# vliu15/3d-brain-tumor-segmentation

Measured on AMD Instinct MI355X. Metric: training volumes/sec (2ch x 128^3), higher is better.
Workload: dtype f32; 1 GPU; BASELINE configs[1]: 2ch x 128^3, batch 1 per GPU, fp32, full fwd+bwd with Dice+KL+L2 VAE loss + Dice metric + TF-form Adam; CLI-default model (base_filters=32, depth=4, groups=8, reduction=8; 42,174,773 params); parallelism=dp1, global_batch=1

## Files before the change

3d-brain-tumor-segmentation_amd/csrc/conv_wgrad.hip:

```cpp
#include <stdlib.h>
#include <type_traits>
#include "common.h"
#include "bts_internal.h"

#define WG_THREADS 512
#define WG_WAVES 8
#define WG_MAXT 4
#define WG_PSLOTS 8
#define WG_QSLOTS 4

struct WgradParams {
  const float* p;
  const float* q;
  float* partial;
  double* partial_b;
  const float* zeros;
  int N, Dp, Hp, Wp, Cp, ldp;
  int Dq, Hq, Wq, Cq, ldq;
  int s, loz, loy, lox;
  int IZ, IY, IX;
  int lgTX, lgTY, TZ;
  int ntz, nty, ntx;
  int ntaps, ntiles, cpad, lgSP;
  int nsub, sub_per_wg;
// ... 467 lines not shown
      float* dst = p.partial + tileBase + (long)(wave + WG_WAVES * i) * 1024;
#pragma unroll
      for (int r = 0; r < 16; ++r) dst[((r & 3) + 8 * (r >> 2) + 4 * h) * 32 + l32] = acc[i][r];
    }
#pragma unroll
    for (int i = 0; i < 3; ++i) {
      __syncthreads();
#pragma unroll
      for (int r = 0; r < 16; ++r) lds[wave * 1024 + ((r & 3) + 8 * (r >> 2) + 4 * h) * 32 + l32] = accx[i][r];
      __syncthreads();
      float* dst = p.partial + tileBase + (long)(24 + i) * 1024;
      for (int e = tid; e < 1024; e += WG_THREADS) {
        float s = lds[e];
#pragma unroll
        for (int w = 1; w < WG_WAVES; ++w) s += lds[w * 1024 + e];
        dst[e] = s;
      }
    }
  } else if (!ksplit) {
#pragma unroll
    for (int i = 0; i < WG_MAXT; ++i) {
      const int tile = wave + WG_WAVES * i;
      if (tile < p.ntiles) {
        float* dst = p.partial + tileBase + (long)tile * 1024;
#pragma unroll
        for (int r = 0; r < 16; ++r) dst[((r & 3) + 8 * (r >> 2) + 4 * h) * 32 + l32] = acc[i][r];
      }
    }
  } else {
#pragma unroll
    for (int i = 0; i < WG_MAXT; ++i) {
      if (i < p.ntiles) {
        __syncthreads();
#pragma unroll
        for (int r = 0; r < 16; ++r) lds[wave * 1024 + ((r & 3) + 8 * (r >> 2) + 4 * h) * 32 + l32] = acc[i][r];
        __syncthreads();
        float* dst = p.partial + tileBase + (long)i * 1024;
        for (int e = tid; e < 1024; e += WG_THREADS) {
          float s = lds[e];
#pragma unroll
          for (int w = 1; w < WG_WAVES; ++w) s += lds[w * 1024 + e];
          dst[e] = s;
        }
      }
    }
  }
  if (p.want_bias && pct == 0) {
    __syncthreads();
    double* shd = reinterpret_cast<double*>(lds);
    shd[tid] = bsum;
    __syncthreads();
    if (tid < 32) {
      double s = 0.0;
      for (int part = 0; part < 16; ++part) s += shd[part * 32 + tid];
      p.partial_b[((long)blockIdx.x * gridDim.z + qct) * 32 + tid] = s;
    }
  }
}

struct WfinParams {
  const float* partial;
  const double* partial_b;
  float* dw;
  float* db;
  int nsp, npct, nqct, ntaps, ntiles, cpad, Cp, Cq;
  long sT, sP, sQ;
  int fold_axis;
  int shift, dup_start;
  int accum;
};

__global__ __launch_bounds__(256) void wgrad_finalize_kernel(const WfinParams f) {
  __shared__ double sh[32][33];
  const int q4 = threadIdx.x & 7, wl = threadIdx.x >> 3;
  const long rows = (long)f.ntaps * f.Cp * f.nqct;
  const long wgStride = (long)f.npct * f.nqct * f.ntiles * 1024;
  for (long row = blockIdx.x; row < rows; row += gridDim.x) {
    const int qct = (int)(row % f.nqct);
    long r = row / f.nqct;
    const int pc = (int)(r % f.Cp);
    const int t = (int)(r / f.Cp);
    long off;
    if (f.cpad == 32) off = ((((long)(pc >> 5)) * f.nqct + qct) * f.ntiles + t) * 1024 + (pc & 31) * 32;
    else {
      const int ci = t * f.cpad + pc;
      off = ((long)qct * f.ntiles + (ci >> 5)) * 1024 + (ci & 31) * 32;
    }
    const float* src = f.partial + off + q4 * 4;
    double s0 = 0.0, s1 = 0.0, s2 = 0.0, s3 = 0.0;
    int w = wl;
    for (; w + 96 < f.nsp; w += 128) {
      const f32x4 a = *reinterpret_cast<const f32x4*>(src + (long)w * wgStride);
      const f32x4 b = *reinterpret_cast<const f32x4*>(src + (long)(w + 32) * wgStride);
      const f32x4 c = *reinterpret_cast<const f32x4*>(src + (long)(w + 64) * wgStride);
      const f32x4 d = *reinterpret_cast<const f32x4*>(src + (long)(w + 96) * wgStride);
      s0 += (double)a[0]; s1 += (double)a[1]; s2 += (double)a[2]; s3 += (double)a[3];
      s0 += (double)b[0]; s1 += (double)b[1]; s2 += (double)b[2]; s3 += (double)b[3];
      s0 += (double)c[0]; s1 += (double)c[1]; s2 += (double)c[2]; s3 += (double)c[3];
      s0 += (double)d[0]; s1 += (double)d[1]; s2 += (double)d[2]; s3 += (double)d[3];
    }
    for (; w < f.nsp; w += 32) {
      const f32x4 a = *reinterpret_cast<const f32x4*>(src + (long)w * wgStride);
      s0 += (double)a[0]; s1 += (double)a[1]; s2 += (double)a[2]; s3 += (double)a[3];
    }
    __syncthreads();
    sh[wl][q4 * 4 + 0] = s0; sh[wl][q4 * 4 + 1] = s1; sh[wl][q4 * 4 + 2] = s2; sh[wl][q4 * 4 + 3] = s3;
    __syncthreads();
    if (threadIdx.x < 32) {
      const int e = threadIdx.x;
      double totd = sh[0][e];
#pragma unroll
      for (int k = 1; k < 32; ++k) totd += sh[k][e];
      const float tot = (float)totd;
      const int qc = qct * 32 + e;
      if (qc < f.Cq) {
        const int pr = (f.fold_axis == 1) ? pc + f.shift : pc;
        const int qr = (f.fold_axis == 2) ? qc + f.shift : qc;
        float* d1 = f.dw + t * f.sT + pr * f.sP + qr * f.sQ;
        *d1 = f.accum ? (*d1 + tot) : tot;
        if (f.shift > 0) {
          if (f.fold_axis == 1 && pc >= f.dup_start) {
            float* d2 = f.dw + t * f.sT + (pc - f.dup_start) * f.sP + qr * f.sQ;
            *d2 = f.accum ? (*d2 + tot) : tot;
          } else if (f.fold_axis == 2 && qc >= f.dup_start) {
            float* d2 = f.dw + t * f.sT + pr * f.sP + (qc - f.dup_start) * f.sQ;
            *d2 = f.accum ? (*d2 + tot) : tot;
          }
        }
      }
    }
  }
  if (f.db && (int)blockIdx.x < f.nqct) {
    const int e = threadIdx.x & 31, l8 = threadIdx.x >> 5, qct = blockIdx.x;
    double s = 0.0;
    for (int w = l8; w < f.nsp; w += 8) s += f.partial_b[((long)w * f.nqct + qct) * 32 + e];
    __syncthreads();
    sh[l8][e] = s;
    __syncthreads();
    if (l8 == 0 && qct * 32 + e < f.Cq) {
      double tot = sh[0][e];
#pragma unroll
      for (int k = 1; k < 8; ++k) tot += sh[k][e];
      const int i = qct * 32 + e;
      f.db[i] = f.accum ? (f.db[i] + (float)tot) : (float)tot;
    }
  }
}

__global__ __launch_bounds__(256) void wgrad_finalize_flat_kernel(const WfinParams f) {
  const int nq = f.nqct * 32;
  const long total = (long)f.ntaps * f.Cp * nq;
  const long wgStride = (long)f.npct * f.nqct * f.ntiles * 1024;
  for (long i = blockIdx.x * (long)blockDim.x + threadIdx.x; i < total; i += (long)gridDim.x * blockDim.x) {
    const int qc = (int)(i % nq);
    long r = i / nq;
    const int pc = (int)(r % f.Cp);
    const int t = (int)(r / f.Cp);
    if (qc >= f.Cq) continue;
    const int qct = qc >> 5, e = qc & 31;
    long off;
    if (f.cpad == 32) off = ((((long)(pc >> 5)) * f.nqct + qct) * f.ntiles + t) * 1024 + (pc & 31) * 32 + e;
    else {
      const int ci = t * f.cpad + pc;
      off = ((long)qct * f.ntiles + (ci >> 5)) * 1024 + (ci & 31) * 32 + e;
    }
    double totd = 0.0;
    for (int w = 0; w < f.nsp; ++w) totd += (double)f.partial[w * wgStride + off];
    const float tot = (float)totd;
    const int pr = (f.fold_axis == 1) ? pc + f.shift : pc;
    const int qr = (f.fold_axis == 2) ? qc + f.shift : qc;
    float* d1 = f.dw + t * f.sT + pr * f.sP + qr * f.sQ;
    *d1 = f.accum ? (*d1 + tot) : tot;
    if (f.shift > 0) {
      if (f.fold_axis == 1 && pc >= f.dup_start) {
        float* d2 = f.dw + t * f.sT + (pc - f.dup_start) * f.sP + qr * f.sQ;
        *d2 = f.accum ? (*d2 + tot) : tot;
      } else if (f.fold_axis == 2 && qc >= f.dup_start) {
        float* d2 = f.dw + t * f.sT + pr * f.sP + (qc - f.dup_start) * f.sQ;
        *d2 = f.accum ? (*d2 + tot) : tot;
      }
    }
  }
  if (f.db && blockIdx.x == 0) {
    for (int i = threadIdx.x; i < f.Cq; i += blockDim.x) {
      double s = 0.0;
      for (int w = 0; w < f.nsp; ++w) s += f.partial_b[((long)w * f.nqct + (i >> 5)) * 32 + (i & 31)];
      f.db[i] = f.accum ? (f.db[i] + (float)s) : (float)s;
    }
  }
}

static int ilog2w(int v) { int l = 0; while ((1 << l) < v) ++l; return l; }

struct WgCall {
  int kind;
  int N, D, H, W;
  int Cin, ldx, Cout, lddy;
  int dup_shift;
  int want_db;
  int x16, dy16;
};
struct WgradRoles {
  int ntaps, s, neg, swapped, transposed;
  int Dp, Hp, Wp, Cp, Dq, Hq, Wq, Cq;
};
struct WgChoice {
  WgradRoles ro;
  WgradParams p;
  int nsp, npct, nqct;
  size_t shmem;
  int variant;
  int sym;
  long NV;
  double flops;
  int clear_zeros;
  long ws_partial, ws_partial_b, ws_colsum, colsum_bytes, ws_zeros, ws;
};

static int plan_wgrad(WgChoice& pl, int ntaps, int s, int neg, int N, int Dp, int Hp, int Wp_, int Cp, int Dq, int Hq,
                      int Wq, int Cq) {
  WgradParams& p = pl.p;
  p.N = N; p.Dp = Dp; p.Hp = Hp; p.Wp = Wp_; p.Cp = Cp;
  p.Dq = Dq; p.Hq = Hq; p.Wq = Wq; p.Cq = Cq;
  p.s = s; p.ntaps = ntaps;
  int lo = 0, span = 1;
  if (ntaps == 27 && s == 1) { lo = -1; span = 3; }
  if (ntaps == 27 && s == 2) { lo = 0; span = 3; }
  p.loz = p.loy = p.lox = lo;
  int cpad = 32;
  if (Cp <= 16 && ntaps == 27) { cpad = 2; while (cpad < Cp) cpad *= 2; }
  p.cpad = cpad;
  const int SP = cpad == 32 ? 32 : (cpad < 4 ? 4 : cpad);
  p.lgSP = ilog2w(SP);
  p.ntiles = (cpad == 32) ? ntaps : (ntaps * cpad + 31) / 32;
  int TX, TY, TZ;
  if (ntaps == 1) { TX = 32; TY = 4; TZ = 2; }
  else if (s == 1) { TX = 16; TY = 4; TZ = 2; }
  else { TX = 8; TY = 4; TZ = 1; }
  while (TX > 2 && TX / 2 >= Wq) { TX /= 2; if (TY * 2 <= 8) TY *= 2; else TZ *= 2; }
  while (TY > 1 && TY / 2 >= Hq) { TY /= 2; TZ *= 2; }
  while (TZ > 1 && TZ / 2 >= Dq && TX * TY * (TZ / 2) >= 2) TZ /= 2;
  p.lgTX = ilog2w(TX); p.lgTY = ilog2w(TY); p.TZ = TZ;
  p.ntx = (Wq + TX - 1) / TX; p.nty = (Hq + TY - 1) / TY; p.ntz = (Dq + TZ - 1) / TZ;
  p.IX = (TX - 1) * s + span; p.IY = (TY - 1) * s + span; p.IZ = (TZ - 1) * s + span;
  const int tileVoxP = p.IZ * p.IY * p.IX;
  const int M = TX * TY * TZ;
  if (tileVoxP * (SP / 4) > WG_THREADS * WG_PSLOTS || M * 8 > WG_THREADS * WG_QSLOTS) return BTS_ERR_SHAPE;
  pl.shmem = (size_t)2 * ((((tileVoxP * (SP / 4) + 63) & ~63) + ((M * 8 + 63) & ~63)) * 4) * sizeof(float);
  if (pl.shmem < (size_t)WG_WAVES * 1024 * sizeof(float)) pl.shmem = (size_t)WG_WAVES * 1024 * sizeof(float);
  if (pl.shmem > 160 * 1024) return BTS_ERR_SHAPE;
  for (int t = 0; t < 27; ++t) p.tap_vox[t] = 0;
  if (ntaps == 27)
    for (int t = 0; t < 27; ++t) {
      int oz = t / 9 + (s == 1 ? -1 : 0), oy = (t / 3) % 3 + (s == 1 ? -1 : 0), ox = t % 3 + (s == 1 ? -1 : 0);
      if (neg) { oz = -oz; oy = -oy; ox = -ox; }
      p.tap_vox[t] = ((oz - lo) * p.IY + (oy - lo)) * p.IX + (ox - lo);
    }
  p.fixg = 0;
  if (ntaps == 27 && cpad == 32 && !neg) {
    if (s == 1 && TX == 16 && TY == 4 && TZ == 2) p.fixg = 1;
    if (s == 2 && TX == 8 && TY == 4 && TZ == 1) p.fixg = 2;
  }
  p.fastf = 0;
  if (p.fixg && Wq % TX == 0 && Hq % TY == 0 && Dq % TZ == 0 && Cp % 32 == 0 && Cq % 32 == 0)
    p.fastf = 1;
  if (!p.fastf) p.fixg = 0;
  p.nsub = N * p.ntz * p.nty * p.ntx;
  pl.npct = (cpad == 32) ? (Cp + 31) / 32 : 1;
  pl.nqct = (Cq + 31) / 32;
  {
    const long pairs = (long)pl.npct * pl.nqct;
    long best = 1;
    double bestc = 1e30;
    long maxn = 2048 / pairs;
    if (maxn < 1) maxn = 1;
    if (maxn > p.nsub) maxn = p.nsub;
    for (long n = 1; n <= maxn; ++n) {
      const long spw = (p.nsub + n - 1) / n;
      const long ne = (p.nsub + spw - 1) / spw;
      if (ne != n) continue;
      const long rounds = (ne * pairs + 255) / 256;
      const double c = (double)rounds * ((double)spw + 0.5) + 0.0023 * (double)(ne * pairs);
      if (c < bestc - 1e-9) { bestc = c; best = n; }
    }
    if (best > p.nsub) best = p.nsub;
    p.sub_per_wg = (int)((p.nsub + best - 1) / best);
    pl.nsp = (p.nsub + p.sub_per_wg - 1) / p.sub_per_wg;
  }
  return BTS_OK;
}

typedef float wg_f32x2 __attribute__((ext_vector_type(2)));
__device__ __forceinline__ wg_f32x2 wgw_pk_add(wg_f32x2 a, wg_f32x2 b) { wg_f32x2 d; asm("v_pk_add_f32 %0, %1, %2" : "=v"(d) : "v"(a), "v"(b)); return d; }
__device__ __forceinline__ wg_f32x2 wgw_pk_sub(wg_f32x2 a, wg_f32x2 b) { wg_f32x2 d; asm("v_pk_add_f32 %0, %1, %2 neg_lo:[0,1] neg_hi:[0,1]" : "=v"(d) : "v"(a), "v"(b)); return d; }
__device__ __forceinline__ wg_f32x2 wgw_pk_fma(wg_f32x2 a, wg_f32x2 b, wg_f32x2 c) { wg_f32x2 d; asm("v_pk_fma_f32 %0, %1, %2, %3" : "=v"(d) : "v"(a), "v"(b), "v"(c)); return d; }
__device__ __forceinline__ wg_f32x2 wgw_pk_addsub(wg_f32x2 a, wg_f32x2 b) { wg_f32x2 d; asm("v_pk_add_f32 %0, %1, %2 op_sel:[0,1] op_sel_hi:[0,1] neg_hi:[0,1]" : "=v"(d) : "v"(a), "v"(b)); return d; }
__device__ __forceinline__ float wgw_acc_rd(float a) { float v; asm volatile("v_accvgpr_read_b32 %0, %1" : "=v"(v) : "a"(a)); return v; }

#define WGW_THREADS 256
#define WGW_RS 18
#define WGW_PTILE (24 * 32 * WGW_RS)
#define WGW_QTILE (8 * 32 * WGW_RS)
#define WGW_BUF (WGW_PTILE + WGW_QTILE)
#define WGW_NPS 14
#define WGW_NQS 4

__global__ __launch_bounds__(WGW_THREADS, 1) void wgw_kernel(const WgradParams p) {
  extern __shared__ __attribute__((aligned(16))) float lds[];
  const int tid = threadIdx.x;
  const int lane = tid & 63;
  const int wave = __builtin_amdgcn_readfirstlane(tid >> 6);
  const int ch = lane & 31, hh = lane >> 5;
  const int pct = blockIdx.y, qct = blockIdx.z;
  const float* pP = p.p + pct * 32;
  const float* pQ = p.q + qct * 32;

  int p_lds[WGW_NPS];
  unsigned poff[WGW_NPS], pfl[3] = {0u, 0u, 0u};
#pragma unroll
  for (int i = 0; i < WGW_NPS; ++i) {
    const int id = tid + WGW_THREADS * i;
    const int idle = id - 24 * 18 * 8;
    p_lds[i] = WGW_PTILE + ((idle >> 4) * 32 + ((idle >> 1) & 7) * 4) * WGW_RS + 16 + (idle & 1);
    poff[i] = 0x80000000u;
    if (id < 24 * 18 * 8) {
      const int cq = id & 7, vox = id >> 3;
      const int row = vox / 18, xx = vox - row * 18;
      const int zr = row / 6, yr = row - zr * 6;
      p_lds[i] = (row * 32 + cq * 4) * WGW_RS + xx;
      poff[i] = (unsigned)(((zr * p.Hp + yr) * p.Wp + xx) * p.ldp + cq * 4) * 4u;
      const unsigned fl = (zr == 0 ? 1u : 0u) | (zr == 3 ? 2u : 0u) | (yr == 0 ? 4u : 0u) | (yr == 5 ? 8u : 0u) |
                          (xx == 0 ? 16u : 0u) | (xx == 17 ? 32u : 0u);
      pfl[i / 5] |= fl << (6 * (i % 5));
    }
  }
  int q_lds[WGW_NQS];
  unsigned qoff[WGW_NQS];
#pragma unroll
  for (int i = 0; i < WGW_NQS; ++i) {
    const int id = tid + WGW_THREADS * i;
    const int cq = id & 7, xx = (id >> 3) & 15, row = id >> 7;
    q_lds[i] = WGW_PTILE + (row * 32 + cq * 4) * WGW_RS + xx;
    qoff[i] = (unsigned)((((row >> 2) * p.Hq + (row & 3)) * p.Wq + xx) * p.ldq + cq * 4) * 4u;
  }
  const int t0 = blockIdx.x * p.sub_per_wg;
  int t1 = t0 + p.sub_per_wg;
  if (t1 > p.nsub) t1 = p.nsub;
  int ftx, fty, ftz, fn;
  {
    int t = t0;
    ftx = t % p.ntx; t /= p.ntx;
    fty = t % p.nty; t /= p.nty;
    ftz = t % p.ntz;
    fn = t / p.ntz;
  }
  f32x4 pre[WGW_NPS + WGW_NQS];
  __amdgpu_buffer_rsrc_t f_pr, f_qr;
  unsigned f_tm = 0;
  auto fetch_begin = [&](bool live) {
    const int z0 = 2 * ftz, y0 = 4 * fty, x0 = 16 * ftx;
    const float* pb = pP + ((((long)fn * p.Dp + z0 - 1) * p.Hp + y0 - 1) * p.Wp + x0 - 1) * p.ldp;
    const float* qb = pQ + ((((long)fn * p.Dq + z0) * p.Hq + y0) * p.Wq + x0) * p.ldq;
    f_pr = __builtin_amdgcn_make_buffer_rsrc((void*)pb, 0, live ? 0x7fffffff : 0, 0x00020000);
    f_qr = __builtin_amdgcn_make_buffer_rsrc((void*)qb, 0, live ? 0x7fffffff : 0, 0x00020000);
    f_tm = (ftz == 0 ? 1u : 0u) | (ftz == p.ntz - 1 ? 2u : 0u) | (fty == 0 ? 4u : 0u) | (fty == p.nty - 1 ? 8u : 0u) |
           (ftx == 0 ? 16u : 0u) | (ftx == p.ntx - 1 ? 32u : 0u);
    const int cx = (ftx + 1 == p.ntx) ? 1 : 0;
    ftx = cx ? 0 : ftx + 1;
    const int cy = (fty + cx == p.nty) ? 1 : 0;
    fty = cy ? 0 : fty + cx;
    const int cz = (ftz + cy == p.ntz) ? 1 : 0;
    ftz = cz ? 0 : ftz + cy;
    fn += cz;
  };
  auto fetch_slot = [&](auto ic) {
    constexpr int i = decltype(ic)::value;
    if constexpr (i < WGW_NPS) {
      const unsigned fl = ((pfl[i / 5] >> (6 * (i % 5))) & 63u) & f_tm;
      pre[i] = __builtin_bit_cast(f32x4, __builtin_amdgcn_raw_buffer_load_b128(f_pr, fl ? 0x80000000u : poff[i], 0, 0));
    } else {
      pre[i] = __builtin_bit_cast(f32x4, __builtin_amdgcn_raw_buffer_load_b128(f_qr, qoff[i - WGW_NPS], 0, 0));
    }
  };
  auto commit_slot = [&](float* buf, auto ic) {
    constexpr int i = decltype(ic)::value;
    if constexpr (i < WGW_NPS) {
#pragma unroll
      for (int e = 0; e < 4; ++e) buf[p_lds[i] + e * WGW_RS] = pre[i][e];
    } else {
#pragma unroll
      for (int e = 0; e < 4; ++e) buf[q_lds[i - WGW_NPS] + e * WGW_RS] = pre[i][e];
    }
  };
  auto fetch_group = [&](auto kc) {
    constexpr int k = decltype(kc)::value;
    fetch_slot(IC<3 * k>{}); fetch_slot(IC<3 * k + 1>{}); fetch_slot(IC<3 * k + 2>{});
  };
  auto commit_group = [&](float* buf, auto kc) {
    constexpr int k = decltype(kc)::value;
    commit_slot(buf, IC<3 * k>{}); commit_slot(buf, IC<3 * k + 1>{}); commit_slot(buf, IC<3 * k + 2>{});
  };

  const int ra = (wave == 0) ? 0 : (wave == 2) ? 2 : 1;
  const int rb = (wave == 0) ? 2 : (wave == 1) ? 2 : (wave == 2) ? 1 : 3;
  const float sp = (wave == 1) ? 1.f : -1.f;
  const wg_f32x2 sp2 = {sp, sp};
  const float sq = (wave == 1) ? 1.f : (wave == 2) ? -1.f : 0.f;
  const wg_f32x2 sq2 = {sq, sq};
  const int pA = (ra * 6 * 32 + ch) * WGW_RS + 2 * hh, pB = (rb * 6 * 32 + ch) * WGW_RS + 2 * hh;
  const int qXa = WGW_PTILE + ((wave == 3 ? 4 : 0) * 32 + ch) * WGW_RS + 2 * hh;
  const int qYa = WGW_PTILE + (4 * 32 + ch) * WGW_RS + 2 * hh;
  const bool bias = p.want_bias && pct == 0 && wave == 1;
  double bsum = 0.0;
  float bs = 0.f;

  f32x16 acc[4][4];
#pragma unroll
  for (int a = 0; a < 4; ++a)
#pragma unroll
    for (int c = 0; c < 4; ++c)
#pragma unroll
      for (int r = 0; r < 16; ++r) acc[a][c][r] = 0.f;

  struct WgwOps { float v[4][4], t[4][4]; };
  auto form = [&](const float* cur, auto stc, WgwOps& o) {
    constexpr int st = decltype(stc)::value;
    constexpr int py = st >> 2, sx = st & 3;
    wg_f32x2 cl[4], cx[4];
#pragma unroll
    for (int yr = 0; yr < 4; ++yr) {
      const float* a = cur + pA + (2 * py + yr) * 32 * WGW_RS + 4 * sx;
      const float* b = cur + pB + (2 * py + yr) * 32 * WGW_RS + 4 * sx;
      cl[yr] = wgw_pk_fma(*reinterpret_cast<const wg_f32x2*>(b), sp2, *reinterpret_cast<const wg_f32x2*>(a));
      cx[yr] = wgw_pk_fma(*reinterpret_cast<const wg_f32x2*>(b + 2), sp2, *reinterpret_cast<const wg_f32x2*>(a + 2));
    }
    wg_f32x2 vl[4], vx[4];
    vl[0] = wgw_pk_sub(cl[0], cl[2]); vx[0] = wgw_pk_sub(cx[0], cx[2]);
    vl[1] = wgw_pk_add(cl[1], cl[2]); vx[1] = wgw_pk_add(cx[1], cx[2]);
    vl[2] = wgw_pk_sub(cl[2], cl[1]); vx[2] = wgw_pk_sub(cx[2], cx[1]);
    vl[3] = wgw_pk_sub(cl[1], cl[3]); vx[3] = wgw_pk_sub(cx[1], cx[3]);
#pragma unroll
    for (int a = 0; a < 4; ++a) {
      const wg_f32x2 d = wgw_pk_sub(vl[a], vx[a]), m = wgw_pk_addsub(vx[a], vl[a]);
      o.v[a][0] = d.x;
      o.v[a][1] = m.x;
      o.v[a][2] = m.y;
      o.v[a][3] = d.y;
    }
    wg_f32x2 qa[2];
#pragma unroll
    for (int yr = 0; yr < 2; ++yr) {
      const wg_f32x2 X = *reinterpret_cast<const wg_f32x2*>(cur + qXa + (2 * py + yr) * 32 * WGW_RS + 4 * sx);
      const wg_f32x2 Y = *reinterpret_cast<const wg_f32x2*>(cur + qYa + (2 * py + yr) * 32 * WGW_RS + 4 * sx);
      qa[yr] = wgw_pk_fma(Y, sq2, X);
    }
    const wg_f32x2 ty[4] = {qa[0], wgw_pk_add(qa[0], qa[1]), wgw_pk_sub(qa[0], qa[1]), qa[1]};
#pragma unroll
    for (int a = 0; a < 4; ++a) {
      const wg_f32x2 m = wgw_pk_addsub(ty[a], ty[a]);
      o.t[a][0] = ty[a].x;
      o.t[a][1] = m.x;
      o.t[a][2] = m.y;
      o.t[a][3] = ty[a].y;
    }
    bs += o.t[1][1];
  };
  auto mfma16 = [&](const WgwOps& o) {
#pragma unroll
    for (int a = 0; a < 4; ++a)
#pragma unroll
      for (int b = 0; b < 4; ++b) acc[a][b] = __builtin_amdgcn_mfma_f32_32x32x2f32(o.v[a][b], o.t[a][b], acc[a][b], 0, 0, 0);
  };
#define WGW_SCHED_STEP()                                   \
  _Pragma("unroll") for (int q_ = 0; q_ < 16; ++q_) {      \
    __builtin_amdgcn_sched_group_barrier(0x008, 1, 0);     \
    __builtin_amdgcn_sched_group_barrier(0x002, 4, 0);     \
    __builtin_amdgcn_sched_group_barrier(0x320, 3, 0);     \
  }
#define WGW_STEP_END()                       \
  WGW_SCHED_STEP();                          \
  __builtin_amdgcn_sched_barrier(0);         \
  asm volatile("s_nop 1" ::: "memory");

  fetch_begin(t0 < t1);
  fetch_group(IC<0>{}); fetch_group(IC<1>{}); fetch_group(IC<2>{}); fetch_group(IC<3>{}); fetch_group(IC<4>{}); fetch_group(IC<5>{});
  commit_group(lds, IC<0>{}); commit_group(lds, IC<1>{}); commit_group(lds, IC<2>{}); commit_group(lds, IC<3>{});
  commit_group(lds, IC<4>{}); commit_group(lds, IC<5>{});
  __syncthreads();
  WgwOps opA, opB;
  form(lds, IC<0>{}, opA);
  fetch_begin((t0 + 1) < t1);
  __builtin_amdgcn_sched_barrier(0);
  asm volatile("s_nop 3" ::: "memory");
  for (int t = t0; t < t1; ++t) {
    const float* cur = lds + ((t - t0) & 1) * WGW_BUF;
    float* nxt = lds + ((t - t0 + 1) & 1) * WGW_BUF;
    form(cur, IC<1>{}, opB); fetch_group(IC<0>{});
    mfma16(opA);
    WGW_STEP_END();
    form(cur, IC<2>{}, opA); commit_group(nxt, IC<0>{}); fetch_group(IC<1>{});
    mfma16(opB);
    WGW_STEP_END();
    form(cur, IC<3>{}, opB); commit_group(nxt, IC<1>{}); fetch_group(IC<2>{});
    mfma16(opA);
    WGW_STEP_END();
    form(cur, IC<4>{}, opA); commit_group(nxt, IC<2>{}); fetch_group(IC<3>{});
    mfma16(opB);
    WGW_STEP_END();
    form(cur, IC<5>{}, opB); commit_group(nxt, IC<3>{}); fetch_group(IC<4>{});
    mfma16(opA);
    WGW_STEP_END();
    form(cur, IC<6>{}, opA); commit_group(nxt, IC<4>{}); fetch_group(IC<5>{});
    mfma16(opB);
    WGW_STEP_END();
    form(cur, IC<7>{}, opB); commit_group(nxt, IC<5>{});
    mfma16(opA);
    WGW_STEP_END();
    bsum += (double)bs;
    bs = 0.f;
    __syncthreads();
    __builtin_amdgcn_sched_barrier(0);
    form(nxt, IC<0>{}, opA);
    fetch_begin((t + 2) < t1);
    mfma16(opB);
    WGW_STEP_END();
  }

  asm volatile("s_nop 15\n\ts_nop 15\n\ts_nop 15\n\ts_nop 15\n\ts_nop 15" ::: "memory");
  __syncthreads();
  float* xl = lds + wave * 9 * 1024;
#pragma unroll
  for (int r = 0; r < 16; ++r) {
    float m[3][4];
#pragma unroll
    for (int b = 0; b < 4; ++b) {
      const float u0 = wgw_acc_rd(acc[0][b][r]), u1 = wgw_acc_rd(acc[1][b][r]), u2 = wgw_acc_rd(acc[2][b][r]),
                  u3 = wgw_acc_rd(acc[3][b][r]);
      const float hs = 0.5f * (u1 + u2), hd = 0.5f * (u1 - u2);
      m[0][b] = u0 + hs;
      m[1][b] = hd;
      m[2][b] = hs - u3;
    }
    const int crow = 8 * (r >> 2) + 4 * hh + (r & 3);
    float* o = xl + crow * 32 + ch;
#pragma unroll
    for (int ky = 0; ky < 3; ++ky) {
      const float hs = 0.5f * (m[ky][1] + m[ky][2]), hd = 0.5f * (m[ky][1] - m[ky][2]);
      o[(ky * 3 + 0) * 1024] = m[ky][0] + hs;
      o[(ky * 3 + 1) * 1024] = hd;
      o[(ky * 3 + 2) * 1024] = hs - m[ky][3];
    }
  }
  __syncthreads();
  float* out = p.partial + ((((long)blockIdx.x * gridDim.y + pct) * gridDim.z + qct) * 27) * 1024;
  for (int e = tid; e < 9 * 1024; e += WGW_THREADS) {
    const float l0 = lds[0 * 9 * 1024 + e], l1 = lds[1 * 9 * 1024 + e], l2 = lds[2 * 9 * 1024 + e], l3 = lds[3 * 9 * 1024 + e];
    const float hs = 0.5f * (l1 + l2), hd = 0.5f * (l1 - l2);
    out[0 * 9 * 1024 + e] = l0 + hs;
    out[1 * 9 * 1024 + e] = hd;
    out[2 * 9 * 1024 + e] = hs - l3;
  }
  if (bias) {
    const double o = __shfl_xor(bsum, 32, 64);
    if (lane < 32) p.partial_b[((long)blockIdx.x * gridDim.z + qct) * 32 + ch] = bsum + o;
  }
}

#define K1W_THREADS 512
#define K1W_U 8
__global__ __launch_bounds__(K1W_THREADS, 2) void k1w_kernel(const WgradParams p, long NV, long chunk) {
  __shared__ float lds[8 * 1024];
  const int tid = threadIdx.x;
  const int lane = tid & 63;
  const int wave = __builtin_amdgcn_readfirstlane(tid >> 6);
  const int ch = lane & 31, hh = lane >> 5;
  const int pct = blockIdx.y, qct = blockIdx.z;
  const int pc = pct * 32 + ch, qc = qct * 32 + ch;
  const bool pok = pc < p.Cp, qok = qc < p.Cq;
  const long w0 = (long)blockIdx.x * chunk;
  long w1 = w0 + chunk;
  if (w1 > NV) w1 = NV;
  long per = ((w1 - w0 + 7) / 8 + 1) & ~1L;
  long v = w0 + wave * per;
  long ve = v + per;
  if (ve > w1) ve = w1;
  f32x16 acc;
#pragma unroll
  for (int r = 0; r < 16; ++r) acc[r] = 0.f;
  double bsum = 0.0;
  const bool bias = p.want_bias && pct == 0;
  const float* pp = p.p + pc;
  const float* qq = p.q + qc;
  for (; v < ve; v += 2 * K1W_U) {
    float a[K1W_U], b[K1W_U];
#pragma unroll
    for (int u = 0; u < K1W_U; ++u) {
      const long vv = v + 2 * u + hh;
      const bool in = vv < ve;
      a[u] = (in && pok) ? pp[vv * p.ldp] : 0.f;
      b[u] = (in && qok) ? qq[vv * p.ldq] : 0.f;
    }
    float bs = 0.f;
#pragma unroll
    for (int u = 0; u < K1W_U; ++u) {
      acc = __builtin_amdgcn_mfma_f32_32x32x2f32(a[u], b[u], acc, 0, 0, 0);
      bs += b[u];
    }
    if (bias) bsum += (double)bs;
  }
#pragma unroll
  for (int r = 0; r < 16; ++r) lds[wave * 1024 + ((r & 3) + 8 * (r >> 2) + 4 * hh) * 32 + ch] = acc[r];
  __syncthreads();
  float* dst = p.partial + ((((long)blockIdx.x * gridDim.y + pct) * gridDim.z + qct) * p.ntiles) * 1024;
  for (int e = tid; e < 1024; e += K1W_THREADS) {
    float sacc = lds[e];
#pragma unroll
    for (int w = 1; w < 8; ++w) sacc += lds[w * 1024 + e];
    dst[e] = sacc;
  }
  if (bias) {
    __syncthreads();
    double* shd = reinterpret_cast<double*>(lds);
    shd[tid] = bsum;
    __syncthreads();
    if (tid < 32) {
      double t = 0.0;
      for (int k = 0; k < 16; ++k) t += shd[k * 32 + tid];
      p.partial_b[((long)blockIdx.x * gridDim.z + qct) * 32 + tid] = t;
    }
  }
}

static int wgrad_roles(WgradRoles& r, int kind, int D, int H, int W, int Cin, int Cout) {
  r.ntaps = (kind == BTS_CONV_K1) ? 1 : 27;
  r.s = 1; r.neg = 0; r.swapped = 0; r.transposed = 0;
  r.Dp = D; r.Hp = H; r.Wp = W; r.Cp = Cin; r.Dq = D; r.Hq = H; r.Wq = W; r.Cq = Cout;
  if (kind == BTS_CONV_K3S2) {
    if ((D | H | W) & 1) return BTS_ERR_SHAPE;
    r.s = 2; r.Dq = D / 2; r.Hq = H / 2; r.Wq = W / 2;
  } else if (kind == BTS_CONV_K3S2T) {
    r.transposed = 1;
    r.s = 2; r.Dp = 2 * D; r.Hp = 2 * H; r.Wp = 2 * W; r.Cp = Cout; r.Cq = Cin;
  } else if (kind == BTS_CONV_K3S1 && Cout <= 8 && Cin > Cout) {
    r.swapped = 1; r.neg = 1; r.Cp = Cout; r.Cq = Cin;
  }
  return BTS_OK;
}

extern "C" int bts_colsum(const float* x, float* out, void* workspace, long workspace_bytes, int N, long rows, int C,
                          int ld, float scale, int sum_over_n, int accumulate, hipStream_t stream);
extern "C" long bts_colsum_workspace(int N, long rows, int C);

static bool wg_switch_on(const char* name) {
  const char* e = getenv(name);
  return !(e && atoi(e) == 0);
}

static int wgrad_choose(const WgCall& c, WgChoice& ch) {
  WgradRoles& ro = ch.ro;
  int r = wgrad_roles(ro, c.kind, c.D, c.H, c.W, c.Cin, c.Cout);
  if (r != BTS_OK) return r;
  if (c.dup_shift > 0 && (c.kind == BTS_CONV_K3S2 || c.kind == BTS_CONV_K3S2T)) return BTS_ERR_UNSUPPORTED;
  r = plan_wgrad(ch, ro.ntaps, ro.s, ro.neg, c.N, ro.Dp, ro.Hp, ro.Wp, ro.Cp, ro.Dq, ro.Hq, ro.Wq, ro.Cq);
  if (r != BTS_OK) return r;
  WgradParams& p = ch.p;
  const bool pIsDy = ro.transposed || ro.swapped;
  p.p = p.q = p.zeros = nullptr; p.partial = nullptr; p.partial_b = nullptr;
  p.ldp = pIsDy ? c.lddy : c.ldx;
  p.ldq = pIsDy ? c.ldx : c.lddy;
  p.want_bias = (c.want_db && !pIsDy) ? 1 : 0;
  ch.ws_partial = 0;
  ch.ws_partial_b = (long)ch.nsp * ch.npct * ch.nqct * p.ntiles * 1024 * 4;
  ch.ws_colsum = (ch.ws_partial_b + (long)ch.nsp * ch.nqct * 32 * 8 + 256 + 15) & ~15L;
  ch.colsum_bytes = ro.swapped ? bts_colsum_workspace(c.N, (long)c.D * c.H * c.W, c.Cout) : 0;
  ch.ws = ch.ws_colsum + ch.colsum_bytes + 128;
  ch.ws_zeros = (ch.ws - 64) & ~15L;
  const bool vec = (p.ldp % 4 == 0) && (p.Cp % 4 == 0) && (p.ldq % 4 == 0) && (p.Cq % 4 == 0) && c.x16 && c.dy16;
  if (p.fastf && ((double)p.IZ * p.Hp * p.Wp * p.ldp * 4.0 >= 4.0e9 || (double)p.TZ * p.Hq * p.Wq * p.ldq * 4.0 >= 4.0e9 || !vec))
    p.fastf = p.fixg = 0;
  ch.variant = !vec ? 0 : (p.fastf ? 1 + p.fixg : 1);
  static const int ksym[4] = {100, 104, 109, 110};
  ch.sym = ksym[ch.variant];
  ch.NV = (long)c.N * ro.Dq * ro.Hq * ro.Wq;
  ch.flops = 2.0 * ro.ntaps * (double)ro.Cp * ro.Cq * (double)ch.NV;
  if (ro.ntaps == 1 && !pIsDy && p.ntiles == 1 && ch.NV >= 32768) {
    if (wg_switch_on("BTS_K1W")) ch.sym = 26;
  } else if (ch.variant == 2 && ro.ntaps == 27 && ro.s == 1 && wg_switch_on("BTS_WGW") &&
             5.0 * p.Hp * p.Wp * p.ldp * 4.0 < 2.0e9 && 3.0 * p.Hq * p.Wq * p.ldq * 4.0 < 2.0e9) {
    ch.sym = 24;
  }
  ch.clear_zeros = ch.sym == 104;
  return BTS_OK;
}

static WgCall wgrad_query_call(int kind, int N, int D, int H, int W, int Cin, int ldx, int Cout, int lddy, int aligned) {
  return WgCall{kind, N, D, H, W, Cin, ldx, Cout, lddy, 0, 0, aligned & 1, (aligned >> 1) & 1};
}

extern "C" long bts_conv3d_bwd_weight_workspace(int kind, int N, int D, int H, int W, int Cin, int Cout) {
  WgChoice ch;
  return wgrad_choose(wgrad_query_call(kind, N, D, H, W, Cin, Cin, Cout, Cout, 3), ch) == BTS_OK ? ch.ws : -1;
}

extern "C" int bts_conv3d_bwd_weight_kernel(int kind, int N, int D, int H, int W, int Cin, int ldx, int Cout, int lddy, int aligned) {
  WgChoice ch;
  const int r = wgrad_choose(wgrad_query_call(kind, N, D, H, W, Cin, ldx, Cout, lddy, aligned), ch);
  return r != BTS_OK ? r : ch.sym;
}

extern "C" int bts_conv3d_bwd_weight_form(int kind, int N, int D, int H, int W, int Cin, int ldx, int Cout, int lddy, int aligned) {
  const int k = bts_conv3d_bwd_weight_kernel(kind, N, D, H, W, Cin, ldx, Cout, lddy, aligned);
  return k < 0 ? k : (k == 24 ? 3 : 0);
}

static int wgrad_launch(const WgChoice& ch, const WgradParams& p, hipStream_t stream) {
  typedef void (*WgKernel)(const WgradParams);
  static const WgKernel kernels[4] = {wgrad_kernel<0, 0>, wgrad_kernel<1, 0>, wgrad_kernel<2, 1>, wgrad_kernel<2, 2>};
  static bool attr_done = false;
  if (!attr_done) {
    for (int i = 0; i < 4; ++i) {
      hipError_t e = hipFuncSetAttribute(reinterpret_cast<const void*>(kernels[i]), hipFuncAttributeMaxDynamicSharedMemorySize, 160 * 1024);
      if (e != hipSuccess) return (int)e;
    }
    attr_done = true;
  }
  if (ch.clear_zeros) {
    hipError_t e = hipMemsetAsync(const_cast<float*>(p.zeros), 0, 64, stream);
    if (e != hipSuccess) return (int)e;
  }
  static bool wattr = false;
  if (ch.sym == 24 && !wattr) {
    hipError_t e = hipFuncSetAttribute(reinterpret_cast<const void*>(wgw_kernel), hipFuncAttributeMaxDynamicSharedMemorySize, 160 * 1024);
    if (e != hipSuccess) return (int)e;
    wattr = true;
  }
  const dim3 grid(ch.nsp, ch.npct, ch.nqct);
  const bool prof = bts_prof_on();
  if (prof) bts_prof_begin(ch.sym, ch.flops, stream);
  (void)hipGetLastError();
  switch (ch.sym) {
    case 26:
      hipLaunchKernelGGL(k1w_kernel, grid, dim3(K1W_THREADS), 0, stream, p, ch.NV, (((ch.NV + ch.nsp - 1) / ch.nsp) + 15) & ~15L);
      break;
    case 24:
      hipLaunchKernelGGL(wgw_kernel, grid, dim3(WGW_THREADS), (size_t)2 * WGW_BUF * sizeof(float), stream, p);
      break;
    default:
      hipLaunchKernelGGL(kernels[ch.variant], grid, dim3(WG_THREADS), ch.shmem, stream, p);
  }
  if (prof) bts_prof_end(stream);
  BTS_LAUNCH_CHECK();
  return BTS_OK;
}

extern "C" int bts_conv3d_bwd_weight(int kind, const float* x, const float* dy, float* dw, float* db, void* workspace,
                                     long workspace_bytes, int N, int D, int H, int W, int Cin, int ldx, int Cout,
                                     int lddy, int dup_start, int dup_shift, int accumulate, hipStream_t stream) {
  const WgCall c{kind, N, D, H, W, Cin, ldx, Cout, lddy, dup_shift, db != nullptr, (((uintptr_t)x) & 15) == 0, (((uintptr_t)dy) & 15) == 0};
  WgChoice ch;
  int r = wgrad_choose(c, ch);
  if (r != BTS_OK) return r;
  if (workspace_bytes < ch.ws || workspace == nullptr) return BTS_ERR_WORKSPACE;
  const WgradRoles& ro = ch.ro;
  const bool pIsDy = ro.transposed || ro.swapped;
  char* ws = reinterpret_cast<char*>(workspace);
  WgradParams p = ch.p;
  p.p = pIsDy ? dy : x;
  p.q = pIsDy ? x : dy;
  p.partial = reinterpret_cast<float*>(ws + ch.ws_partial);
  p.partial_b = reinterpret_cast<double*>(((uintptr_t)(ws + ch.ws_partial_b) + 15) & ~(uintptr_t)15);
  p.zeros = reinterpret_cast<const float*>(ws + ch.ws_zeros);
  r = wgrad_launch(ch, p, stream);
  if (r != BTS_OK) return r;
  WfinParams f;
  f.partial = p.partial; f.partial_b = p.partial_b; f.dw = dw; f.db = p.want_bias ? db : nullptr;
  f.nsp = ch.nsp; f.npct = ch.npct; f.nqct = ch.nqct; f.ntaps = ro.ntaps; f.ntiles = p.ntiles; f.cpad = p.cpad;
  f.Cp = ro.Cp; f.Cq = ro.Cq;
  const int Cin_ref = Cin + dup_shift;
  f.sT = (long)Cin_ref * Cout;
  if (ro.transposed) { f.sP = Cin_ref; f.sQ = 1; f.fold_axis = 0; }
  else if (ro.swapped) { f.sP = 1; f.sQ = Cout; f.fold_axis = 2; }
  else { f.sP = Cout; f.sQ = 1; f.fold_axis = 1; }
  f.shift = dup_shift;
  f.dup_start = dup_shift > 0 ? dup_start : (1 << 30);
  f.accum = accumulate;
  long rows = (long)ro.ntaps * ro.Cp * ch.nqct;
  if (ch.nsp <= 16) {
    long blocks = (rows * 32 + 255) / 256;
    if (blocks > 8192) blocks = 8192;
    (void)hipGetLastError(); hipLaunchKernelGGL(wgrad_finalize_flat_kernel, dim3((int)blocks), dim3(256), 0, stream, f);
  } else {
    int blocks = (int)(rows < 4096 ? rows : 4096);
    (void)hipGetLastError(); hipLaunchKernelGGL(wgrad_finalize_kernel, dim3(blocks), dim3(256), 0, stream, f);
  }
  BTS_LAUNCH_CHECK();
  if (db != nullptr && ro.swapped)
    return bts_colsum(dy, db, ws + ch.ws_colsum, ch.colsum_bytes, N, (long)D * H * W, Cout, lddy, 1.0f, 1, accumulate, stream);
  return BTS_OK;
}
```

Before: 28.95 volumes/s.

## Pre-transform z-planes at commit time and deepen wgrad fetch/LDS-read pipeline

The Winograd-style z-direction input transform moves from the per-step LDS read path into the global-to-LDS commit. Each thread loads the four z rows of a voxel column and stores the four transformed planes, so each wave reads one pre-combined plane instead of two rows plus an FMA. LDS reads (rd) are split from the arithmetic transform (xf) and software-pipelined one step ahead, and global fetches for the next tile now start earlier using incrementally advanced pointers with per-plane buffer descriptors for boundary masking. This cuts LDS read traffic and VALU work in the MFMA loop, at the cost of more live registers, a different boundary-masking scheme and a moved barrier placement.

```diff
diff --git a/3d-brain-tumor-segmentation_amd/csrc/conv_wgrad.hip b/3d-brain-tumor-segmentation_amd/csrc/conv_wgrad.hip
--- a/3d-brain-tumor-segmentation_amd/csrc/conv_wgrad.hip
+++ b/3d-brain-tumor-segmentation_amd/csrc/conv_wgrad.hip
@@ -793,7 +793,8 @@
 #define WGW_PTILE (24 * 32 * WGW_RS)
 #define WGW_QTILE (8 * 32 * WGW_RS)
 #define WGW_BUF (WGW_PTILE + WGW_QTILE)
-#define WGW_NPS 14
+#define WGW_PLANE (6 * 32 * WGW_RS)
+#define WGW_NPC 4
 #define WGW_NQS 4
 
 __global__ __launch_bounds__(WGW_THREADS, 1) void wgw_kernel(const WgradParams p) {
@@ -806,23 +807,28 @@
   const float* pP = p.p + pct * 32;
   const float* pQ = p.q + qct * 32;
 
-  int p_lds[WGW_NPS];
-  unsigned poff[WGW_NPS], pfl[3] = {0u, 0u, 0u};
-#pragma unroll
-  for (int i = 0; i < WGW_NPS; ++i) {
+  int c_lds[WGW_NPC - 1], c3_lds[4];
+  unsigned coff[WGW_NPC], cfl = 0u;
+#pragma unroll
+  for (int i = 0; i < WGW_NPC; ++i) {
     const int id = tid + WGW_THREADS * i;
-    const int idle = id - 24 * 18 * 8;
-    p_lds[i] = WGW_PTILE + ((idle >> 4) * 32 + ((idle >> 1) & 7) * 4) * WGW_RS + 16 + (idle & 1);
-    poff[i] = 0x80000000u;
-    if (id < 24 * 18 * 8) {
+    int l = 0;
+    coff[i] = 0x80000000u;
+    if (id < 6 * 18 * 8) {
       const int cq = id & 7, vox = id >> 3;
-      const int row = vox / 18, xx = vox - row * 18;
-      const int zr = row / 6, yr = row - zr * 6;
-      p_lds[i] = (row * 32 + cq * 4) * WGW_RS + xx;
-      poff[i] = (unsigned)(((zr * p.Hp + yr) * p.Wp + xx) * p.ldp + cq * 4) * 4u;
-      const unsigned fl = (zr == 0 ? 1u : 0u) | (zr == 3 ? 2u : 0u) | (yr == 0 ? 4u : 0u) | (yr == 5 ? 8u : 0u) |
-                          (xx == 0 ? 16u : 0u) | (xx == 17 ? 32u : 0u);
-      pfl[i / 5] |= fl << (6 * (i % 5));
+      const int yr = vox / 18, xx = vox - yr * 18;
+      l = (yr * 32 + cq * 4) * WGW_RS + xx;
+      coff[i] = (unsigned)((yr * p.Wp + xx) * p.ldp + cq * 4) * 4u;
+      const unsigned fl = (yr == 0 ? 1u : 0u) | (yr == 5 ? 2u : 0u) | (xx == 0 ? 4u : 0u) | (xx == 17 ? 8u : 0u);
+      cfl |= fl << (4 * i);
+    }
+    if (i < WGW_NPC - 1) {
+      c_lds[i < WGW_NPC - 1 ? i : 0] = l;
+    } else {
+      const int idle = id - 6 * 18 * 8;
+#pragma unroll
+      for (int pl = 0; pl < 4; ++pl)
+        c3_lds[pl] = idle < 0 ? l + pl * WGW_PLANE : WGW_PTILE + 4 * (((idle >> 1) + 16 * pl) & 63) * WGW_RS + 16 + (idle & 1);
     }
   }
   int q_lds[WGW_NQS];
@@ -845,60 +851,89 @@
     ftz = t % p.ntz;
     fn = t / p.ntz;
   }
-  f32x4 pre[WGW_NPS + WGW_NQS];
-  __amdgpu_buffer_rsrc_t f_pr, f_qr;
-  unsigned f_tm = 0;
+  const char* f_pb = reinterpret_cast<const char*>(pP + ((((long)fn * p.Dp + 2 * ftz - 1) * p.Hp + 4 * fty - 1) * p.Wp + 16 * ftx - 1) * p.ldp);
+  const char* f_qb = reinterpret_cast<const char*>(pQ + ((((long)fn * p.Dq + 2 * ftz) * p.Hq + 4 * fty) * p.Wq + 16 * ftx) * p.ldq);
+  const long zrow = (long)p.Hp * p.Wp * p.ldp;
+  const unsigned pdx = 64u * p.ldp, pdy = 12u * p.Wp * p.ldp, pdz = (unsigned)zrow * 4u;
+  const unsigned qdx = 64u * p.ldq, qdy = 12u * p.Wq * p.ldq, qdz = (unsigned)p.Hq * p.Wq * p.ldq * 4u;
+  f32x4 pre[4 * WGW_NPC + WGW_NQS];
+  __amdgpu_buffer_rsrc_t f_pr[4], f_qr;
+  unsigned f_cm[WGW_NPC] = {0u, 0u, 0u, 0u};
   auto fetch_begin = [&](bool live) {
-    const int z0 = 2 * ftz, y0 = 4 * fty, x0 = 16 * ftx;
-    const float* pb = pP + ((((long)fn * p.Dp + z0 - 1) * p.Hp + y0 - 1) * p.Wp + x0 - 1) * p.ldp;
-    const float* qb = pQ + ((((long)fn * p.Dq + z0) * p.Hq + y0) * p.Wq + x0) * p.ldq;
-    f_pr = __builtin_amdgcn_make_buffer_rsrc((void*)pb, 0, live ? 0x7fffffff : 0, 0x00020000);
+    const float* pb = reinterpret_cast<const float*>(f_pb);
+    const float* qb = reinterpret_cast<const float*>(f_qb);
+    f_pr[0] = __builtin_amdgcn_make_buffer_rsrc((void*)pb, 0, (live && ftz != 0) ? 0x7fffffff : 0, 0x00020000);
+    f_pr[1] = __builtin_amdgcn_make_buffer_rsrc((void*)(pb + zrow), 0, live ? 0x7fffffff : 0, 0x00020000);
+    f_pr[2] = __builtin_amdgcn_make_buffer_rsrc((void*)(pb + 2 * zrow), 0, live ? 0x7fffffff : 0, 0x00020000);
+    f_pr[3] = __builtin_amdgcn_make_buffer_rsrc((void*)(pb + 3 * zrow), 0, (live && ftz != p.ntz - 1) ? 0x7fffffff : 0, 0x00020000);
     f_qr = __builtin_amdgcn_make_buffer_rsrc((void*)qb, 0, live ? 0x7fffffff : 0, 0x00020000);
-    f_tm = (ftz == 0 ? 1u : 0u) | (ftz == p.ntz - 1 ? 2u : 0u) | (fty == 0 ? 4u : 0u) | (fty == p.nty - 1 ? 8u : 0u) |
-           (ftx == 0 ? 16u : 0u) | (ftx == p.ntx - 1 ? 32u : 0u);
+    const unsigned tm = (fty == 0 ? 1u : 0u) | (fty == p.nty - 1 ? 2u : 0u) | (ftx == 0 ? 4u : 0u) | (ftx == p.ntx - 1 ? 8u : 0u);
+#pragma unroll
+    for (int i = 0; i < WGW_NPC; ++i) f_cm[i] = tm << (4 * i);
     const int cx = (ftx + 1 == p.ntx) ? 1 : 0;
     ftx = cx ? 0 : ftx + 1;
     const int cy = (fty + cx == p.nty) ? 1 : 0;
     fty = cy ? 0 : fty + cx;
     const int cz = (ftz + cy == p.ntz) ? 1 : 0;
     ftz = cz ? 0 : ftz + cy;
-    fn += cz;
-  };
-  auto fetch_slot = [&](auto ic) {
-    constexpr int i = decltype(ic)::value;
-    if constexpr (i < WGW_NPS) {
-      const unsigned fl = ((pfl[i / 5] >> (6 * (i % 5))) & 63u) & f_tm;
-      pre[i] = __builtin_bit_cast(f32x4, __builtin_amdgcn_raw_buffer_load_b128(f_pr, fl ? 0x80000000u : poff[i], 0, 0));
-    } else {
-      pre[i] = __builtin_bit_cast(f32x4, __builtin_amdgcn_raw_buffer_load_b128(f_qr, qoff[i - WGW_NPS], 0, 0));
-    }
-  };
-  auto commit_slot = [&](float* buf, auto ic) {
-    constexpr int i = decltype(ic)::value;
-    if constexpr (i < WGW_NPS) {
-#pragma unroll
-      for (int e = 0; e < 4; ++e) buf[p_lds[i] + e * WGW_RS] = pre[i][e];
-    } else {
-#pragma unroll
-      for (int e = 0; e < 4; ++e) buf[q_lds[i - WGW_NPS] + e * WGW_RS] = pre[i][e];
-    }
+    f_pb += pdx + cx * pdy + cy * pdz;
+    f_qb += qdx + cx * qdy + cy * qdz;
+  };
+  auto load4 = [](__amdgpu_buffer_rsrc_t r, unsigned off) {
+    return __builtin_bit_cast(f32x4, __builtin_amdgcn_raw_buffer_load_b128(r, off, 0, 0));
+  };
+  auto sub4 = [](f32x4 a, f32x4 b) {
+    const wg_f32x2 lo = wgw_pk_sub(a.xy, b.xy), hi = wgw_pk_sub(a.zw, b.zw);
+    return f32x4{lo.x, lo.y, hi.x, hi.y};
+  };
+  auto add4 = [](f32x4 a, f32x4 b) {
+    const wg_f32x2 lo = wgw_pk_add(a.xy, b.xy), hi = wgw_pk_add(a.zw, b.zw);
+    return f32x4{lo.x, lo.y, hi.x, hi.y};
   };
   auto fetch_group = [&](auto kc) {
     constexpr int k = decltype(kc)::value;
-    fetch_slot(IC<3 * k>{}); fetch_slot(IC<3 * k + 1>{}); fetch_slot(IC<3 * k + 2>{});
+    if constexpr (k < WGW_NPC) {
+      const unsigned off = (cfl & f_cm[k]) ? 0x80000000u : coff[k];
+#pragma unroll
+      for (int zr = 0; zr < 4; ++zr) pre[4 * k + zr] = load4(f_pr[zr], off);
+    } else {
+      constexpr int i = 2 * (k - WGW_NPC);
+      pre[4 * WGW_NPC + i] = load4(f_qr, qoff[i]);
+      pre[4 * WGW_NPC + i + 1] = load4(f_qr, qoff[i + 1]);
+    }
   };
   auto commit_group = [&](float* buf, auto kc) {
     constexpr int k = decltype(kc)::value;
-    commit_slot(buf, IC<3 * k>{}); commit_slot(buf, IC<3 * k + 1>{}); commit_slot(buf, IC<3 * k + 2>{});
-  };
-
-  const int ra = (wave == 0) ? 0 : (wave == 2) ? 2 : 1;
-  const int rb = (wave == 0) ? 2 : (wave == 1) ? 2 : (wave == 2) ? 1 : 3;
-  const float sp = (wave == 1) ? 1.f : -1.f;
-  const wg_f32x2 sp2 = {sp, sp};
+    if constexpr (k < WGW_NPC) {
+      const f32x4 d0 = pre[4 * k], d1 = pre[4 * k + 1], d2 = pre[4 * k + 2], d3 = pre[4 * k + 3];
+      const f32x4 pl[4] = {sub4(d0, d2), add4(d1, d2), sub4(d2, d1), sub4(d1, d3)};
+#pragma unroll
+      for (int z = 0; z < 4; ++z) {
+        float* o;
+        if constexpr (k < WGW_NPC - 1) o = buf + c_lds[k] + z * WGW_PLANE;
+        else o = buf + c3_lds[z];
+#pragma unroll
+        for (int e = 0; e < 4; ++e) o[e * WGW_RS] = pl[z][e];
+      }
+    } else {
+      constexpr int i0 = 2 * (k - WGW_NPC);
+#pragma unroll
+      for (int i = i0; i < i0 + 2; ++i)
+#pragma unroll
+        for (int e = 0; e < 4; ++e) buf[q_lds[i] + e * WGW_RS] = pre[4 * WGW_NPC + i][e];
+    }
+  };
+  auto stage = [&](float* buf, auto sc, bool live2) {
+    constexpr int s = decltype(sc)::value;
+    if constexpr (s <= 5) commit_group(buf, IC<s>{});
+    if constexpr (s == 6) fetch_begin(live2);
+    if constexpr (s + 2 <= 5) fetch_group(IC<s + 2>{});
+    else if constexpr (s >= 6) fetch_group(IC<s - 6>{});
+  };
+
   const float sq = (wave == 1) ? 1.f : (wave == 2) ? -1.f : 0.f;
   const wg_f32x2 sq2 = {sq, sq};
-  const int pA = (ra * 6 * 32 + ch) * WGW_RS + 2 * hh, pB = (rb * 6 * 32 + ch) * WGW_RS + 2 * hh;
+  const int pA = wave * WGW_PLANE + ch * WGW_RS + 2 * hh;
   const int qXa = WGW_PTILE + ((wave == 3 ? 4 : 0) * 32 + ch) * WGW_RS + 2 * hh;
   const int qYa = WGW_PTILE + (4 * 32 + ch) * WGW_RS + 2 * hh;
   const bool bias = p.want_bias && pct == 0 && wave == 1;
@@ -914,22 +949,28 @@
       for (int r = 0; r < 16; ++r) acc[a][c][r] = 0.f;
 
   struct WgwOps { float v[4][4], t[4][4]; };
-  auto form = [&](const float* cur, auto stc, WgwOps& o) {
+  struct WgwRaw { wg_f32x2 pl[4], px[4], qx[2], qy[2]; };
+  auto rd = [&](const float* cur, auto stc, WgwRaw& r) {
     constexpr int st = decltype(stc)::value;
     constexpr int py = st >> 2, sx = st & 3;
-    wg_f32x2 cl[4], cx[4];
 #pragma unroll
     for (int yr = 0; yr < 4; ++yr) {
       const float* a = cur + pA + (2 * py + yr) * 32 * WGW_RS + 4 * sx;
-      const float* b = cur + pB + (2 * py + yr) * 32 * WGW_RS + 4 * sx;
-      cl[yr] = wgw_pk_fma(*reinterpret_cast<const wg_f32x2*>(b), sp2, *reinterpret_cast<const wg_f32x2*>(a));
-      cx[yr] = wgw_pk_fma(*reinterpret_cast<const wg_f32x2*>(b + 2), sp2, *reinterpret_cast<const wg_f32x2*>(a + 2));
-    }
+      r.pl[yr] = *reinterpret_cast<const wg_f32x2*>(a);
+      r.px[yr] = *reinterpret_cast<const wg_f32x2*>(a + 2);
+    }
+#pragma unroll
+    for (int yr = 0; yr < 2; ++yr) {
+      r.qx[yr] = *reinterpret_cast<const wg_f32x2*>(cur + qXa + (2 * py + yr) * 32 * WGW_RS + 4 * sx);
+      r.qy[yr] = *reinterpret_cast<const wg_f32x2*>(cur + qYa + (2 * py + yr) * 32 * WGW_RS + 4 * sx);
+    }
+  };
+  auto xf = [&](const WgwRaw& r, WgwOps& o) {
     wg_f32x2 vl[4], vx[4];
-    vl[0] = wgw_pk_sub(cl[0], cl[2]); vx[0] = wgw_pk_sub(cx[0], cx[2]);
-    vl[1] = wgw_pk_add(cl[1], cl[2]); vx[1] = wgw_pk_add(cx[1], cx[2]);
-    vl[2] = wgw_pk_sub(cl[2], cl[1]); vx[2] = wgw_pk_sub(cx[2], cx[1]);
-    vl[3] = wgw_pk_sub(cl[1], cl[3]); vx[3] = wgw_pk_sub(cx[1], cx[3]);
+    vl[0] = wgw_pk_sub(r.pl[0], r.pl[2]); vx[0] = wgw_pk_sub(r.px[0], r.px[2]);
+    vl[1] = wgw_pk_add(r.pl[1], r.pl[2]); vx[1] = wgw_pk_add(r.px[1], r.px[2]);
+    vl[2] = wgw_pk_sub(r.pl[2], r.pl[1]); vx[2] = wgw_pk_sub(r.px[2], r.px[1]);
+    vl[3] = wgw_pk_sub(r.pl[1], r.pl[3]); vx[3] = wgw_pk_sub(r.px[1], r.px[3]);
 #pragma unroll
     for (int a = 0; a < 4; ++a) {
       const wg_f32x2 d = wgw_pk_sub(vl[a], vx[a]), m = wgw_pk_addsub(vx[a], vl[a]);
@@ -938,13 +979,7 @@
       o.v[a][2] = m.y;
       o.v[a][3] = d.y;
     }
-    wg_f32x2 qa[2];
-#pragma unroll
-    for (int yr = 0; yr < 2; ++yr) {
-      const wg_f32x2 X = *reinterpret_cast<const wg_f32x2*>(cur + qXa + (2 * py + yr) * 32 * WGW_RS + 4 * sx);
-      const wg_f32x2 Y = *reinterpret_cast<const wg_f32x2*>(cur + qYa + (2 * py + yr) * 32 * WGW_RS + 4 * sx);
-      qa[yr] = wgw_pk_fma(Y, sq2, X);
-    }
+    const wg_f32x2 qa[2] = {wgw_pk_fma(r.qy[0], sq2, r.qx[0]), wgw_pk_fma(r.qy[1], sq2, r.qx[1])};
     const wg_f32x2 ty[4] = {qa[0], wgw_pk_add(qa[0], qa[1]), wgw_pk_sub(qa[0], qa[1]), qa[1]};
 #pragma unroll
     for (int a = 0; a < 4; ++a) {
@@ -979,40 +1014,49 @@
   commit_group(lds, IC<4>{}); commit_group(lds, IC<5>{});
   __syncthreads();
   WgwOps opA, opB;
-  form(lds, IC<0>{}, opA);
+  WgwRaw rawA, rawB;
+  rd(lds, IC<0>{}, rawA);
+  __builtin_amdgcn_sched_barrier(0);
   fetch_begin((t0 + 1) < t1);
+  fetch_group(IC<0>{});
+  __builtin_amdgcn_sched_barrier(0);
+  rd(lds, IC<1>{}, rawB);
+  __builtin_amdgcn_sched_barrier(0);
+  xf(rawA, opA);
+  __builtin_amdgcn_sched_barrier(0);
+  fetch_group(IC<1>{});
   __builtin_amdgcn_sched_barrier(0);
   asm volatile("s_nop 3" ::: "memory");
   for (int t = t0; t < t1; ++t) {
     const float* cur = lds + ((t - t0) & 1) * WGW_BUF;
     float* nxt = lds + ((t - t0 + 1) & 1) * WGW_BUF;
-    form(cur, IC<1>{}, opB); fetch_group(IC<0>{});
+    const bool live2 = (t + 2) < t1;
+    rd(cur, IC<2>{}, rawA); xf(rawB, opB); stage(nxt, IC<0>{}, live2);
     mfma16(opA);
     WGW_STEP_END();
-    form(cur, IC<2>{}, opA); commit_group(nxt, IC<0>{}); fetch_group(IC<1>{});
+    rd(cur, IC<3>{}, rawB); xf(rawA, opA); stage(nxt, IC<1>{}, live2);
     mfma16(opB);
     WGW_STEP_END();
-    form(cur, IC<3>{}, opB); commit_group(nxt, IC<1>{}); fetch_group(IC<2>{});
+    rd(cur, IC<4>{}, rawA); xf(rawB, opB); stage(nxt, IC<2>{}, live2);
     mfma16(opA);
     WGW_STEP_END();
-    form(cur, IC<4>{}, opA); commit_group(nxt, IC<2>{}); fetch_group(IC<3>{});
+    rd(cur, IC<5>{}, rawB); xf(rawA, opA); stage(nxt, IC<3>{}, live2);
     mfma16(opB);
     WGW_STEP_END();
-    form(cur, IC<5>{}, opB); commit_group(nxt, IC<3>{}); fetch_group(IC<4>{});
+    rd(cur, IC<6>{}, rawA); xf(rawB, opB); stage(nxt, IC<4>{}, live2);
     mfma16(opA);
     WGW_STEP_END();
-    form(cur, IC<6>{}, opA); commit_group(nxt, IC<4>{}); fetch_group(IC<5>{});
+    rd(cur, IC<7>{}, rawB); xf(rawA, opA); stage(nxt, IC<5>{}, live2);
     mfma16(opB);
     WGW_STEP_END();
-    form(cur, IC<7>{}, opB); commit_group(nxt, IC<5>{});
+    __syncthreads();
+    __builtin_amdgcn_sched_barrier(0);
+    rd(nxt, IC<0>{}, rawA); xf(rawB, opB); stage(nxt, IC<6>{}, live2);
     mfma16(opA);
     WGW_STEP_END();
     bsum += (double)bs;
     bs = 0.f;
-    __syncthreads();
-    __builtin_amdgcn_sched_barrier(0);
-    form(nxt, IC<0>{}, opA);
-    fetch_begin((t + 2) < t1);
+    rd(nxt, IC<1>{}, rawB); xf(rawA, opA); stage(nxt, IC<7>{}, live2);
     mfma16(opB);
     WGW_STEP_END();
   }
```

New measurement: 29.45 volumes/s, median of 6. +1.7%, better.
